# BarclayII/audiogan

Hardware: AMD Instinct MI355X
Metric: audio-samples/sec per G+D train step (8 kHz, 8192-sample clips) (higher is better)
Workload: dtype f32; 1 GPU; C2: full audiogan.py Conv1d/LSTM G + D, batch 64 per GPU, 8192-sample white-noise clips, frame_size 256 (T=32), canonical G+D step, adam, per-parameter clip d=1 g=0.1; global_batch=64, clip_len=8192, parallelism=dp1, launch=hipGraph replay (1 graph per step)

## Files before the change

audiogan_amd/csrc/conv_grad.hip:

```cpp
#include "common.h"

struct WgP {
  const float* sh;
  const float* lg;
  float* dw;
  int64_t sh_bs, sh_cs, lg_bs, lg_cs;
  int B, A, Lsh, C, Llg, K, s, p;
  int CK;
  int TC;
  int nchunk;
  int lgp;
  int maxch;
  int vec;
  float* part;
  int rb;
};

template <int TA, int TN, int WA, int WN>
__global__ __launch_bounds__(512) void conv_wgrad_kernel(const WgP p) {
  int bx = blockIdx.x, by = blockIdx.y, bz = blockIdx.z;
  const int gz_ = gridDim.z;
  {
    const int gx = gridDim.x, gy = gridDim.y, nwg = gx * gy * gz_;
    if (nwg >= 16) {
      const int lin = (bz * gy + by) * gx + bx;
      const int xi = lin & 7, q = nwg >> 3, r = nwg & 7;
      const int t = xi * q + (xi < r ? xi : r) + (lin >> 3);
      bx = t % gx; by = (t / gx) % gy; bz = t / (gx * gy);
    }
  }
  static_assert(WA * WN == 4, "4 compute waves");
  constexpr int AT = 32 * TA * WA, NT = 32 * TN * WN;
  constexpr int SP = AT + 1;
  extern __shared__ float smem[];
  const size_t bufsz = (size_t)p.TC * SP + (size_t)p.maxch * p.lgp;

  const int tid = threadIdx.x, lane = tid & 63, wid = tid >> 6;
  const int l31 = lane & 31, h = lane >> 5;
  const int cw = wid & 3;
  const int wa = cw / WN, wn = cw % WN;
  const int a0 = by * AT, ck0 = bx * NT;
  const int c_lo = ck0 / p.K;
  int c_hi = (ck0 + NT - 1) / p.K;
  if (c_hi >= p.C) c_hi = p.C - 1;
  const int nch = c_hi - c_lo + 1;
  const int span = p.s * (p.TC - 1) + p.K;
  const int total = p.B * p.nchunk;
  const int nmine = (total - bz + gz_ - 1) / gz_;

  auto stage = [&](int ch, int buf, int sw, int nsw) {
    float* shs = smem + buf * bufsz;
    float* lgs = shs + (size_t)p.TC * SP;
    const int b = ch / p.nchunk;
    const int t0 = (ch - b * p.nchunk) * p.TC;
    const float* sb = p.sh + (int64_t)b * p.sh_bs;
    const float* lb = p.lg + (int64_t)b * p.lg_bs;
    const int g0 = p.s * t0 - p.p;
    const int q4 = p.TC >> 2;
    const int stot = AT * q4, ltot = nch * span, step = nsw * 64;
    constexpr int US = 4, UL = 4;
    int se = sw * 64 + lane, le = se;
    while (se < stot || le < ltot) {
      f32x4 sv[US];
      float lv[UL];
#pragma unroll
      for (int u = 0; u < US; ++u) {
        const int e = se + u * step;
        sv[u] = f32x4{0.f, 0.f, 0.f, 0.f};
        if (e < stot) {
          const int r = e / q4, q = e - r * q4;
          const int a = a0 + r, tg = t0 + 4 * q;
          if (a < p.A) {
            const float* src = sb + (int64_t)a * p.sh_cs + tg;
            if (p.vec && tg + 3 < p.Lsh) {
              sv[u] = *reinterpret_cast<const f32x4*>(src);
            } else {
#pragma unroll
              for (int x = 0; x < 4; ++x)
                if (tg + x < p.Lsh) sv[u][x] = src[x];
            }
          }
        }
      }
#pragma unroll
      for (int u = 0; u < UL; ++u) {
        const int e = le + u * step;
        lv[u] = 0.f;
        if (e < ltot) {
          const int r = e / span, i = e - r * span;
          const int g = g0 + i;
          if (g >= 0 && g < p.Llg) lv[u] = lb[(int64_t)(c_lo + r) * p.lg_cs + g];
        }
      }
      if (p.rb) {
#pragma unroll
        for (int u = 0; u < US; ++u) sv[u] = ag_rbf4_if(sv[u], 1);
#pragma unroll
        for (int u = 0; u < UL; ++u) lv[u] = ag_rbf(lv[u]);
      }
#pragma unroll
      for (int u = 0; u < US; ++u) {
        const int e = se + u * step;
        if (e < stot) {
          const int r = e / q4, q = e - r * q4;
#pragma unroll
          for (int x = 0; x < 4; ++x) shs[(4 * q + x) * SP + r] = sv[u][x];
        }
      }
#pragma unroll
      for (int u = 0; u < UL; ++u) {
        const int e = le + u * step;
        if (e < ltot) {
          const int r = e / span, i = e - r * span;
          lgs[r * p.lgp + i] = lv[u];
        }
      }
      se += US * step;
      le += UL * step;
    }
  };

  if (nmine > 0) stage(bz, 0, wid, 8);
  __syncthreads();

  if (__builtin_amdgcn_readfirstlane(threadIdx.x) >= 256) {
    __builtin_amdgcn_s_setprio(2);
    constexpr int FS = 4, FL = 5;
    const int shift = (((-p.p) % 4) + 4) % 4;
    const int PR = (shift + span + 3) / 4;
    const int q4 = p.TC >> 2;
    const int stot = AT * q4, ltot4 = nch * PR;
    const bool fastp = p.vec && (p.Lsh % p.TC == 0) && ((p.s * p.TC) % 4 == 0) && (p.Llg % 4 == 0) && p.Llg >= 4 &&
                       (p.lg_cs % 4 == 0) && (p.lg_bs % 4 == 0) && (((uintptr_t)p.lg & 15) == 0) &&
                       stot <= FS * 256 && ltot4 <= FL * 256 && (int64_t)AT * p.sh_cs < (1 << 30) &&
                       (int64_t)p.maxch * p.lg_cs < (1 << 30);
    int ssrc[FS], sl[FS], lsrc[FL], li0[FL], lrow[FL];
    if (fastp) {
#pragma unroll
      for (int u = 0; u < FS; ++u) {
        const int e = cw * 64 + lane + u * 256;
        const int r = e / q4, q = e - r * q4;
        const bool ok = e < stot && a0 + r < p.A;
        ssrc[u] = ok ? (int)((a0 + r) * p.sh_cs) + 4 * q : 0;
        sl[u] = e < stot ? (4 * q) * SP + r : -1;
        if (e < stot && !ok) ssrc[u] = -1;
      }
#pragma unroll
      for (int u = 0; u < FL; ++u) {
        const int e = cw * 64 + lane + u * 256;
        const int r = e / PR, m = e - r * PR;
        const bool ok = e < ltot4;
        lsrc[u] = ok ? (int)((c_lo + r) * p.lg_cs) + 4 * m : 0;
        li0[u] = ok ? 4 * m - shift : -(1 << 20);
        lrow[u] = r * p.lgp;
      }
    }
    int ci = 0;
    if (fastp) {
      for (; ci < nmine; ++ci) {
        if (ci + 1 < nmine) {
          const int ch = bz + (ci + 1) * gz_;
          const int b = ch / p.nchunk;
          const int t0 = (ch - b * p.nchunk) * p.TC;
          const int g0 = p.s * t0 - p.p;
          float* shs = smem + ((ci + 1) & 1) * bufsz;
          float* lgs = shs + (size_t)p.TC * SP;
          const float* sbase = p.sh + (int64_t)b * p.sh_bs + t0;
          const float* lrow0 = p.lg + (int64_t)b * p.lg_bs;
          f32x4 sv[FS], lv[FL];
          bool lok[FL];
#pragma unroll
          for (int u = 0; u < FS; ++u) sv[u] = *reinterpret_cast<const f32x4*>(sbase + max(ssrc[u], 0));
#pragma unroll
          for (int u = 0; u < FL; ++u) {
            const int gp = g0 + li0[u];
            lok[u] = gp >= 0 && gp + 3 < p.Llg;
            lv[u] = *reinterpret_cast<const f32x4*>(lrow0 + (lok[u] ? lsrc[u] + (g0 - shift) : 0));
          }
          if (p.rb) {
#pragma unroll
            for (int u = 0; u < FS; ++u) sv[u] = ag_rbf4_if(sv[u], 1);
#pragma unroll
            for (int u = 0; u < FL; ++u) lv[u] = ag_rbf4_if(lv[u], 1);
          }
#pragma unroll
          for (int u = 0; u < FS; ++u)
            if (sl[u] >= 0) {
#pragma unroll
              for (int x = 0; x < 4; ++x) shs[sl[u] + x * SP] = ssrc[u] < 0 ? 0.f : sv[u][x];
            }
#pragma unroll
          for (int u = 0; u < FL; ++u)
#pragma unroll
            for (int x = 0; x < 4; ++x) {
              const int i = li0[u] + x;
              if (i >= 0 && i < span) lgs[lrow[u] + i] = lok[u] ? lv[u][x] : 0.f;
            }
        }
        __syncthreads();
      }
    }
    for (; ci < nmine; ++ci) {
      if (ci + 1 < nmine) stage(bz + (ci + 1) * gz_, (ci + 1) & 1, cw, 4);
      __syncthreads();
    }
    return;
  }

  int joff[TN];
  bool jok[TN];
#pragma unroll
  for (int j = 0; j < TN; ++j) {
    const int ck = ck0 + wn * 32 * TN + 32 * j + l31;
    jok[j] = ck < p.CK;
    const int c = jok[j] ? ck / p.K : c_lo;
    const int k = jok[j] ? ck - c * p.K : 0;
    joff[j] = (c - c_lo) * p.lgp + k + p.s * h;
  }
  f32x16 acc[TA][TN];
#pragma unroll
  for (int i = 0; i < TA; ++i)
#pragma unroll
    for (int j = 0; j < TN; ++j)
#pragma unroll
      for (int e = 0; e < 16; ++e) acc[i][j][e] = 0.f;

  for (int ci = 0; ci < nmine; ++ci) {
    const float* shs = smem + (ci & 1) * bufsz;
    const float* lgs = shs + (size_t)p.TC * SP;
    const float* arow = shs + h * SP + wa * 32 * TA + l31;
    for (int t = 0; t < p.TC; t += 2) {
      float av[TA], bv[TN];
#pragma unroll
      for (int i = 0; i < TA; ++i) av[i] = arow[t * SP + 32 * i];
#pragma unroll
      for (int j = 0; j < TN; ++j) {
        const float bval = lgs[joff[j] + p.s * t];
        bv[j] = jok[j] ? bval : 0.f;
      }
#pragma unroll
      for (int i = 0; i < TA; ++i)
#pragma unroll
        for (int j = 0; j < TN; ++j)
          acc[i][j] = __builtin_amdgcn_mfma_f32_32x32x2f32(av[i], bv[j], acc[i][j], 0, 0, 0);
    }
    __syncthreads();
  }

#pragma unroll
  for (int i = 0; i < TA; ++i)
#pragma unroll
    for (int e = 0; e < 16; ++e) {
      const int a = a0 + wa * 32 * TA + 32 * i + (e & 3) + 8 * (e >> 2) + 4 * h;
      if (a >= p.A) continue;
#pragma unroll
      for (int j = 0; j < TN; ++j) {
        const int ck = ck0 + wn * 32 * TN + 32 * j + l31;
        if (ck >= p.CK) continue;
        p.part[((int64_t)bz * p.A + a) * p.CK + ck] = acc[i][j][e];
      }
    }
}

typedef short wbf16x8 __attribute__((ext_vector_type(8)));
typedef unsigned wu32x4 __attribute__((ext_vector_type(4)));
typedef unsigned wu32x2 __attribute__((ext_vector_type(2)));
#define WB_FS 8
#define WB_FL 5

template <int TA, int TN, int WA, int WN>
__global__ __launch_bounds__(512) void conv_wgrad_bf16_kernel(const WgP p) {
  int bx = blockIdx.x, by = blockIdx.y, bz = blockIdx.z;
  const int gz_ = gridDim.z;
  {
    const int gx = gridDim.x, gy = gridDim.y, nwg = gx * gy * gz_;
    if (nwg >= 16) {
      const int lin = (bz * gy + by) * gx + bx;
      const int xi = lin & 7, q = nwg >> 3, r = nwg & 7;
      const int t = xi * q + (xi < r ? xi : r) + (lin >> 3);
      bx = t % gx; by = (t / gx) % gy; bz = t / (gx * gy);
    }
  }
  static_assert(WA * WN == 4, "4 compute waves");
  constexpr int AT = 32 * TA * WA, NT = 32 * TN * WN;
  extern __shared__ float smem[];
  char* lds = reinterpret_cast<char*>(smem);
  const int SPB = p.TC * 2 + 16;
  const int LGPB = p.lgp;
  const size_t bufb = ((size_t)AT * SPB + (size_t)p.maxch * LGPB + 15) & ~(size_t)15;

  const int tid = threadIdx.x, lane = tid & 63, wid = tid >> 6;
  const int l31 = lane & 31, h = lane >> 5;
  const int cw = wid & 3;
  const int wa = cw / WN, wn = cw % WN;
  const int a0 = by * AT, ck0 = bx * NT;
  const int c_lo = ck0 / p.K;
  int c_hi = (ck0 + NT - 1) / p.K;
  if (c_hi >= p.C) c_hi = p.C - 1;
  const int nch = c_hi - c_lo + 1;
  const int span = p.s * (p.TC - 1) + p.K;
  const int total = p.B * p.nchunk;
  const int nmine = (total - bz + gz_ - 1) / gz_;

  if (__builtin_amdgcn_readfirstlane(threadIdx.x) >= 256) {
    __builtin_amdgcn_s_setprio(2);
    const int sl_ = cw * 64 + lane;
    const int shift = (((-p.p) % 4) + 4) % 4;
    const int PR = (shift + span + 3) / 4;
    const int q4 = p.TC >> 2;
    const int stot = AT * q4, ltot4 = nch * PR;
    int ssrc[WB_FS], sdst[WB_FS], lsrc[WB_FL], li0[WB_FL], lrow[WB_FL];
#pragma unroll
    for (int u = 0; u < WB_FS; ++u) {
      const int e = sl_ + u * 256;
      const int r = e / q4, q = e - r * q4;
      const bool ok = e < stot && a0 + r < p.A;
      ssrc[u] = ok ? (int)((a0 + r) * p.sh_cs) + 4 * q : -1;
      sdst[u] = e < stot ? r * SPB + 8 * q : -1;
    }
#pragma unroll
    for (int u = 0; u < WB_FL; ++u) {
      const int e = sl_ + u * 256;
      const int r = e / PR, m = e - r * PR;
      const bool ok = e < ltot4;
      lsrc[u] = ok ? (int)((c_lo + r) * p.lg_cs) + 4 * m : 0;
      li0[u] = ok ? 4 * m - shift : -(1 << 20);
      lrow[u] = r * LGPB;
    }
    f32x4 sv[WB_FS], lv[WB_FL];
    bool lok[WB_FL];
    auto loadc = [&](int cix) __attribute__((always_inline)) {
      const int ch = bz + cix * gz_;
      const int b = ch / p.nchunk;
      const int t0 = (ch - b * p.nchunk) * p.TC;
      const int g0 = p.s * t0 - p.p;
      const float* sbase = p.sh + (int64_t)b * p.sh_bs + t0;
      const float* lrow0 = p.lg + (int64_t)b * p.lg_bs;
#pragma unroll
      for (int u = 0; u < WB_FS; ++u) sv[u] = *reinterpret_cast<const f32x4*>(sbase + max(ssrc[u], 0));
#pragma unroll
      for (int u = 0; u < WB_FL; ++u) {
        const int gp = g0 + li0[u];
        lok[u] = gp >= 0 && gp + 3 < p.Llg;
        lv[u] = *reinterpret_cast<const f32x4*>(lrow0 + (lok[u] ? lsrc[u] + (g0 - shift) : 0));
      }
    };
    auto writec = [&](int buf) __attribute__((always_inline)) {
      char* shs = lds + buf * bufb;
      char* lgs = shs + (size_t)AT * SPB;
#pragma unroll
      for (int u = 0; u < WB_FS; ++u)
        if (sdst[u] >= 0) {
          wu32x2 w = {ag_pack_bf16(sv[u][0], sv[u][1]), ag_pack_bf16(sv[u][2], sv[u][3])};
          if (ssrc[u] < 0) w = wu32x2{0u, 0u};
          *reinterpret_cast<wu32x2*>(shs + sdst[u]) = w;
        }
#pragma unroll
      for (int u = 0; u < WB_FL; ++u)
#pragma unroll
        for (int x = 0; x < 4; ++x) {
          const int i = li0[u] + x;
          if (i >= 0 && i < span)
            *reinterpret_cast<unsigned short*>(lgs + lrow[u] + 2 * i) = lok[u] ? (unsigned short)ag_pack_bf16(lv[u][x], lv[u][x]) : (unsigned short)0;
        }
    };
    if (nmine > 0) {
      loadc(0);
      writec(0);
    }
    __builtin_amdgcn_sched_barrier(0);
    if (nmine > 1) loadc(1);
    __syncthreads();
    for (int ci = 0; ci < nmine; ++ci) {
      if (ci + 1 < nmine) writec((ci + 1) & 1);
      __builtin_amdgcn_sched_barrier(0);
      if (ci + 2 < nmine) loadc(ci + 2);
      __syncthreads();
    }
    return;
  }

  int joff[TN];
  bool jok[TN];
#pragma unroll
  for (int j = 0; j < TN; ++j) {
    const int ck = ck0 + wn * 32 * TN + 32 * j + l31;
    jok[j] = ck < p.CK;
    const int c = jok[j] ? ck / p.K : c_lo;
    const int k = jok[j] ? ck - c * p.K : 0;
    joff[j] = (c - c_lo) * LGPB + 2 * (k + p.s * 8 * h);
  }
  f32x16 acc[TA][TN];
#pragma unroll
  for (int i = 0; i < TA; ++i)
#pragma unroll
    for (int j = 0; j < TN; ++j)
#pragma unroll
      for (int e = 0; e < 16; ++e) acc[i][j][e] = 0.f;
  __syncthreads();
  const int s2 = 2 * p.s;
  for (int ci = 0; ci < nmine; ++ci) {
    const char* shs = lds + (ci & 1) * bufb;
    const char* lgs = shs + (size_t)AT * SPB;
    const char* arow = shs + (size_t)(wa * 32 * TA + l31) * SPB + 16 * h;
    for (int tb = 0; tb < p.TC; tb += 16) {
      wbf16x8 av[TA], bv[TN];
#pragma unroll
      for (int i = 0; i < TA; ++i) av[i] = *reinterpret_cast<const wbf16x8*>(arow + (size_t)32 * i * SPB + 2 * tb);
#pragma unroll
      for (int j = 0; j < TN; ++j) {
        const char* bp = lgs + joff[j] + s2 * tb;
        wu32x4 w;
#pragma unroll
        for (int e = 0; e < 4; ++e) {
          const unsigned lo = *reinterpret_cast<const unsigned short*>(bp + s2 * (2 * e));
          const unsigned hi = *reinterpret_cast<const unsigned short*>(bp + s2 * (2 * e + 1));
          w[e] = jok[j] ? (lo | (hi << 16)) : 0u;
        }
        bv[j] = __builtin_bit_cast(wbf16x8, w);
      }
#pragma unroll
      for (int i = 0; i < TA; ++i)
#pragma unroll
        for (int j = 0; j < TN; ++j)
          acc[i][j] = __builtin_amdgcn_mfma_f32_32x32x16_bf16(av[i], bv[j], acc[i][j], 0, 0, 0);
    }
    __syncthreads();
  }

#pragma unroll
  for (int i = 0; i < TA; ++i)
#pragma unroll
    for (int e = 0; e < 16; ++e) {
      const int a = a0 + wa * 32 * TA + 32 * i + (e & 3) + 8 * (e >> 2) + 4 * h;
      if (a >= p.A) continue;
#pragma unroll
      for (int j = 0; j < TN; ++j) {
        const int ck = ck0 + wn * 32 * TN + 32 * j + l31;
        if (ck >= p.CK) continue;
        p.part[((int64_t)bz * p.A + a) * p.CK + ck] = acc[i][j][e];
      }
    }
}

static int wgrad_slices(int A, int CK, int AT, int NT, int total) {
  const int gx = ag_cdiv(CK, NT), gy = ag_cdiv(A, AT);
  int gz = ag_cdiv(512, gx * gy);
  if (gz > total) gz = total;
  if (gz < 1) gz = 1;
  return gz;
}

template <int TA, int TN, int WA, int WN>
static int launch_wgrad_bf16(WgP& p, hipStream_t st, AgWs ws) {
  constexpr int AT = 32 * TA * WA, NT = 32 * TN * WN;
  p.TC = 64;
  if (p.Lsh % p.TC != 0 || !p.vec || (p.s * p.TC) % 4 != 0 || p.Llg % 4 != 0 || p.Llg < 4 || p.lg_cs % 4 != 0 ||
      p.lg_bs % 4 != 0 || (((uintptr_t)p.lg) & 15) != 0)
    return -1;
  p.nchunk = p.Lsh / p.TC;
  const int span = p.s * (p.TC - 1) + p.K;
  p.lgp = ag_roundup(2 * span, 4) + 4;
  p.maxch = (NT - 1) / p.K + 2;
  if (p.maxch > p.C) p.maxch = p.C;
  const int shift = (((-p.p) % 4) + 4) % 4;
  const int PR = (shift + span + 3) / 4;
  if (AT * (p.TC / 4) > WB_FS * 256 || p.maxch * PR > WB_FL * 256) return -1;
  if ((int64_t)AT * p.sh_cs >= (1 << 30) || (int64_t)p.C * p.lg_cs >= (1 << 30)) return -1;
  const size_t lds = 2 * (((size_t)AT * (p.TC * 2 + 16) + (size_t)p.maxch * p.lgp + 15) & ~(size_t)15);
  if (lds > 160 * 1024) return -1;
  const int gx = ag_cdiv(p.CK, NT), gy = ag_cdiv(p.A, AT);
  const int total = p.B * p.nchunk;
  int gz = wgrad_slices(p.A, p.CK, AT, NT, total);
  const int64_t n_out = (int64_t)p.A * p.CK;
  AG_REQUIRE(ws.p && ws.numel >= n_out, "%s: this reduction spans several workgroups and needs a workspace of >= %lld floats bound with ag_bind_workspace (sums are two-stage, in a fixed order; there is no float-atomic accumulation)", "ag_conv1d_wgrad", (long long)n_out);
  if ((int64_t)gz * n_out > ws.numel) gz = (int)(ws.numel / n_out);
  p.part = ws.p;
  auto kern = conv_wgrad_bf16_kernel<TA, TN, WA, WN>;
  if (lds > 64 * 1024)
    (void)hipFuncSetAttribute((const void*)kern, hipFuncAttributeMaxDynamicSharedMemorySize, (int)lds);
  static const AgKernelName name("conv_wgrad_bf16_kernel", {TA, TN, WA, WN});
  ag_note_kernel(name.s);
  hipLaunchKernelGGL(kern, dim3(gx, gy, gz), dim3(512), lds, st, p);
  AG_CHECK_LAUNCH("ag_conv1d_wgrad(bf16)");
  return ag_slab_reduce(p.part, gz, n_out, p.dw, 1, st);
}

template <int TA, int TN, int WA, int WN>
static int launch_wgrad(WgP& p, hipStream_t st, AgWs ws) {
  constexpr int AT = 32 * TA * WA, NT = 32 * TN * WN;
  if (p.rb) {
    const int rc = launch_wgrad_bf16<TA, TN, WA, WN>(p, st, ws);
    if (rc != -1) return rc;
  }
  p.TC = AT >= 128 ? 32 : 64;
  if (p.Lsh < p.TC) p.TC = ag_roundup(p.Lsh, 4);
  p.nchunk = ag_cdiv(p.Lsh, p.TC);
  const int span = p.s * (p.TC - 1) + p.K;
  p.lgp = span | 1;
  p.maxch = (NT - 1) / p.K + 2;
  if (p.maxch > p.C) p.maxch = p.C;
  const size_t lds = 2 * ((size_t)p.TC * (AT + 1) + (size_t)p.maxch * p.lgp) * sizeof(float);
  if (lds > 160 * 1024) {
    ag_set_error("conv wgrad: tile needs %zu B of LDS", lds);
    return AG_ERR_UNSUPPORTED;
  }
  const int gx = ag_cdiv(p.CK, NT), gy = ag_cdiv(p.A, AT);
  const int total = p.B * p.nchunk;
  int gz = wgrad_slices(p.A, p.CK, AT, NT, total);
  const int64_t n_out = (int64_t)p.A * p.CK;
  AG_REQUIRE(ws.p && ws.numel >= n_out, "%s: this reduction spans several workgroups and needs a workspace of >= %lld floats bound with ag_bind_workspace (sums are two-stage, in a fixed order; there is no float-atomic accumulation)", "ag_conv1d_wgrad", (long long)n_out);
  if ((int64_t)gz * n_out > ws.numel) gz = (int)(ws.numel / n_out);
  p.part = ws.p;
  auto kern = conv_wgrad_kernel<TA, TN, WA, WN>;
  if (lds > 64 * 1024)
    (void)hipFuncSetAttribute((const void*)kern, hipFuncAttributeMaxDynamicSharedMemorySize,
                              (int)lds);
  static const AgKernelName name("conv_wgrad_kernel", {TA, TN, WA, WN});
  ag_note_kernel(name.s);
  hipLaunchKernelGGL(kern, dim3(gx, gy, gz), dim3(512), lds, st, p);
  AG_CHECK_LAUNCH("ag_conv1d_wgrad");
  return ag_slab_reduce(p.part, gz, n_out, p.dw, 1, st);
}

template <int KMAX, int AG>
__global__ __launch_bounds__(256) void conv_c1_wgrad_kernel(const float* __restrict__ sh, int64_t sh_bs, int64_t sh_cs,
                                                            const float* __restrict__ lg, int64_t lg_bs,
                                                            float* __restrict__ dw, int B, int A, int Lsh, int Llg,
                                                            int K, int s, int p, int bper, float* __restrict__ part,
                                                            int rb) {
  __shared__ float red[4][AG * KMAX];
  const int a0 = blockIdx.y * AG;
  const int t = blockIdx.x * 256 + threadIdx.x;
  const int b0 = blockIdx.z * bper, b1 = min(B, b0 + bper);
  float acc[AG][KMAX];
#pragma unroll
  for (int i = 0; i < AG; ++i)
#pragma unroll
    for (int k = 0; k < KMAX; ++k) acc[i][k] = 0.f;
  if (t < Lsh) {
    const int q0 = s * t - p;
    for (int b = b0; b < b1; ++b) {
      const float* xr = lg + (int64_t)b * lg_bs;
      float win[KMAX];
#pragma unroll
      for (int k = 0; k < KMAX; ++k) {
        const int q = q0 + k;
        const float xv = xr[min(max(q, 0), Llg - 1)];
        win[k] = (k < K && q >= 0 && q < Llg) ? ag_rbf_if(xv, rb) : 0.f;
      }
      const float* dyr = sh + (int64_t)b * sh_bs + t;
#pragma unroll
      for (int i = 0; i < AG; ++i) {
        const float g = ag_rbf_if(dyr[(int64_t)min(a0 + i, A - 1) * sh_cs], rb);
#pragma unroll
        for (int k = 0; k < KMAX; ++k) acc[i][k] += g * win[k];
      }
    }
  }
#pragma unroll
  for (int i = 0; i < AG; ++i)
#pragma unroll
    for (int k = 0; k < KMAX; ++k) {
      const float v = ag_wave_sum(acc[i][k]);
      if ((threadIdx.x & 63) == 0) red[threadIdx.x >> 6][i * KMAX + k] = v;
    }
  __syncthreads();
  if (threadIdx.x < AG * KMAX) {
    const int i = threadIdx.x / KMAX, k = threadIdx.x % KMAX;
    if (k < K && a0 + i < A) {
      const float v = red[0][threadIdx.x] + red[1][threadIdx.x] + red[2][threadIdx.x] + red[3][threadIdx.x];
      part[((int64_t)(blockIdx.z * gridDim.x + blockIdx.x) * A + a0 + i) * K + k] = v;
    }
  }
}

extern "C" int ag_conv1d_wgrad(const float* sh, int64_t sh_bs, int64_t sh_cs, const float* lg,
                               int64_t lg_bs, int64_t lg_cs, float* dw, int B, int A, int Lsh, int C,
                               int Llg, int K, int stride, int pad, void* stream) {
  const AgWs ws = ag_ws_take();
  AG_REQUIRE(sh && lg && dw, "ag_conv1d_wgrad: null tensor");
  AG_REQUIRE(B > 0 && A > 0 && Lsh > 0 && C > 0 && Llg > 0 && K > 0 && stride > 0 && pad >= 0,
             "ag_conv1d_wgrad: bad shape");
  WgP p;
  p.sh = sh; p.lg = lg; p.dw = dw;
  p.sh_bs = sh_bs; p.sh_cs = sh_cs; p.lg_bs = lg_bs; p.lg_cs = lg_cs;
  p.B = B; p.A = A; p.Lsh = Lsh; p.C = C; p.Llg = Llg; p.K = K; p.s = stride; p.p = pad;
  p.CK = C * K;
  p.rb = ag_precision() == AG_PREC_BF16;
  p.vec = (((uintptr_t)sh & 15) == 0) && (sh_bs % 4 == 0) && (sh_cs % 4 == 0);
  hipStream_t st = (hipStream_t)stream;
  if (C == 1 && ws.p && ag_conv_c1_wgrad_slabs(B, A, Lsh, stride, K, nullptr) > 0 &&
      (((uintptr_t)sh & 15) == 0) && sh_bs % 4 == 0 && sh_cs % 4 == 0 &&
      ws.numel >= (int64_t)ag_conv_c1_wgrad_slabs(B, A, Lsh, stride, K, nullptr) * A * K &&
      ag_conv_c1_enabled()) {
    const int slabs = ag_conv_c1_wgrad_slabs(B, A, Lsh, stride, K, nullptr);
    const int rc = ag_conv_c1_wgrad(sh, sh_bs, sh_cs, lg, lg_bs, ws.p, B, A, Lsh, Llg, stride, K, pad, p.rb, st);
    if (rc != AG_OK) return rc;
    return ag_slab_reduce(ws.p, slabs, (int64_t)A * K, dw, 1, st);
  }
  if (C == 1 && K <= 8) {
    const int ag = 8;
    const int gx = ag_cdiv(Lsh, 256), gy = ag_cdiv(A, ag);
    int gz = ag_cdiv(512, gx * gy);
    if (gz > B) gz = B;
    if (gz < 1) gz = 1;
    AG_REQUIRE(ws.p && ws.numel >= (int64_t)gx * A * K, "%s: this reduction spans several workgroups and needs a workspace of >= %lld floats bound with ag_bind_workspace (sums are two-stage, in a fixed order; there is no float-atomic accumulation)", "ag_conv1d_wgrad", (long long)gx * A * K);
    if ((int64_t)gz * gx * A * K > ws.numel) gz = (int)(ws.numel / ((int64_t)gx * A * K));
    float* part = ws.p;
    const int bper = ag_cdiv(B, gz);
    gz = ag_cdiv(B, bper);
    ag_note_kernel("conv_c1_wgrad_kernel<8,8>");
    hipLaunchKernelGGL((conv_c1_wgrad_kernel<8, 8>), dim3(gx, gy, gz), dim3(256), 0, st, sh, sh_bs, sh_cs, lg, lg_bs,
                       dw, B, A, Lsh, Llg, K, stride, pad, bper, part, p.rb);
    AG_CHECK_LAUNCH("ag_conv1d_wgrad");
    return ag_slab_reduce(part, gx * gz, (int64_t)A * K, dw, 1, st);
  }
  if (A <= 32) return launch_wgrad<1, 1, 1, 4>(p, st, ws);
  if (A <= 64 || p.CK <= 64) return launch_wgrad<1, 1, 2, 2>(p, st, ws);
  return launch_wgrad<2, 2, 2, 2>(p, st, ws);
}

extern "C" int64_t ag_conv1d_wgrad_ws_numel(int B, int A, int Lsh, int C, int K) {
  if (C == 1 && K == 7) {
    const int64_t need = (int64_t)ag_conv_c1_wgrad_slabs(B, A, Lsh, 2, K, nullptr) * A * K;
    const int gx = ag_cdiv(Lsh, 256), gy = ag_cdiv(A, 8);
    int gz = ag_cdiv(512, gx * gy);
    if (gz > B) gz = B;
    if (gz < 1) gz = 1;
    const int64_t n2 = (int64_t)gz * gx * A * K;
    return n2 > need ? n2 : need;
  }
  if (C == 1 && K <= 8) {
    const int gx = ag_cdiv(Lsh, 256), gy = ag_cdiv(A, 8);
    int gz = ag_cdiv(512, gx * gy);
    if (gz > B) gz = B;
    if (gz < 1) gz = 1;
    return (int64_t)gz * gx * A * K;
  }
  const int CK = C * K;
  int AT, NT;
  if (A <= 32) { AT = 32; NT = 128; }
  else if (A <= 64 || CK <= 64) { AT = 64; NT = 64; }
  else { AT = 128; NT = 128; }
  int TC = AT >= 128 ? 32 : 64;
  if (Lsh < TC) TC = ag_roundup(Lsh, 4);
  const int total = B * ag_cdiv(Lsh, TC);
  return (int64_t)wgrad_slices(A, CK, AT, NT, total) * A * CK;
}

__global__ __launch_bounds__(256) void channel_sum_kernel(const float* __restrict__ dy, int64_t bs,
                                                          int64_t cs, float* __restrict__ db, int B,
                                                          int C, int L, int nsplit, float* __restrict__ part, int accumulate) {
  __shared__ float red[17];
  const int c = blockIdx.x;
  const int64_t total = (int64_t)B * L;
  float s = 0.f;
  for (int64_t i = (int64_t)blockIdx.y * 256 + threadIdx.x; i < total; i += (int64_t)nsplit * 256) {
    const int b = (int)(i / L);
    const int t = (int)(i - (int64_t)b * L);
    s += dy[(int64_t)b * bs + (int64_t)c * cs + t];
  }
  s = ag_block_sum(s, red);
  if (threadIdx.x == 0) {
    if (part) part[(int64_t)blockIdx.y * C + c] = s;
    else db[c] = accumulate ? db[c] + s : s;
  }
}

extern "C" int ag_channel_sum(const float* dy, int64_t bs, int64_t cs, float* db, int B, int C, int L, int accumulate,
                              void* stream) {
  const AgWs ws = ag_ws_take();
  AG_REQUIRE(dy && db && B > 0 && C > 0 && L > 0, "ag_channel_sum: bad args");
  int nsplit = (int)ag_cdiv64((int64_t)B * L, 256 * 16);
  const int cap = ag_cdiv(2048, C);
  if (nsplit > cap) nsplit = cap;
  if (nsplit < 1) nsplit = 1;
  float* part = nullptr;
  if (nsplit > 1) {
    AG_REQUIRE(ws.p && ws.numel >= 2 * (int64_t)C, "%s: this reduction spans several workgroups and needs a workspace of >= %lld floats bound with ag_bind_workspace (sums are two-stage, in a fixed order; there is no float-atomic accumulation)", "ag_channel_sum", (long long)2 * C);
    if ((int64_t)nsplit * C > ws.numel) nsplit = (int)(ws.numel / C);
    part = ws.p;
  }
  hipLaunchKernelGGL(channel_sum_kernel, dim3(C, nsplit), dim3(256), 0, (hipStream_t)stream, dy, bs,
                     cs, db, B, C, L, nsplit, part, accumulate);
  AG_CHECK_LAUNCH("ag_channel_sum");
  if (part) return ag_slab_reduce(part, nsplit, C, db, accumulate ? 1 : 0, (hipStream_t)stream);
  return AG_OK;
}

__global__ __launch_bounds__(256) void leaky_bwd_kernel(const float* __restrict__ dy, int64_t dy_bs,
                                                        int64_t dy_cs, const float* __restrict__ y,
                                                        int64_t y_bs, int64_t y_cs,
                                                        float* __restrict__ dp, int64_t dp_bs,
                                                        int64_t dp_cs, float* __restrict__ ad,
                                                        int64_t ad_bs, int64_t ad_cs,
                                                        const int64_t* __restrict__ lens,
                                                        float* __restrict__ bias_grad, int B, int C,
                                                        int L, int bper, float slope, float* __restrict__ part) {
  const int c = blockIdx.y;
  float bsum = 0.f;
  for (int b = blockIdx.z * bper; b < min(B, (int)(blockIdx.z + 1) * bper); ++b) {
    const int64_t lenb = lens ? lens[b] : (int64_t)1 << 60;
    const float* dyr = dy + (int64_t)b * dy_bs + (int64_t)c * dy_cs;
    const float* yr = y + (int64_t)b * y_bs + (int64_t)c * y_cs;
    float* dpr = dp + (int64_t)b * dp_bs + (int64_t)c * dp_cs;
    float* adr = ad ? ad + (int64_t)b * ad_bs + (int64_t)c * ad_cs : nullptr;
    for (int t = blockIdx.x * 256 + threadIdx.x; t < L; t += gridDim.x * 256) {
      float g = dyr[t];
      g = (yr[t] > 0.f) ? g : g * slope;
      if (t >= lenb) g = 0.f;
      dpr[t] = g;
      if (adr) adr[t] += g;
      bsum += g;
    }
  }
  if (bias_grad) {
    __shared__ float red[4];
    bsum = ag_wave_sum(bsum);
    if ((threadIdx.x & 63) == 0) red[threadIdx.x >> 6] = bsum;
    __syncthreads();
    if (threadIdx.x == 0) {
      const float v = red[0] + red[1] + red[2] + red[3];
      part[(int64_t)(blockIdx.z * gridDim.x + blockIdx.x) * C + c] = v;
    }
  }
}

extern "C" int ag_leaky_bwd(const float* dy, int64_t dy_bs, int64_t dy_cs, const float* y,
                            int64_t y_bs, int64_t y_cs, float* dpre, int64_t dp_bs, int64_t dp_cs,
                            float* add_into, int64_t ad_bs, int64_t ad_cs, const int64_t* lens_i64,
                            float* bias_grad, int B, int C, int L, float slope, void* stream) {
  const AgWs ws = ag_ws_take();
  AG_REQUIRE(dy && y && dpre && B > 0 && C > 0 && L > 0, "ag_leaky_bwd: bad args");
  AG_REQUIRE(B <= 65535 && C <= 65535, "ag_leaky_bwd: B or C > 65535");
  int gx = ag_cdiv(L, 256 * 4);
  if (gx < 1) gx = 1;
  int bper = 1;
  float* part = nullptr;
  if (bias_grad) {
    bper = (int)(((int64_t)gx * C * B) / 2048);
    if (bper < 8) bper = 8;
    if (bper > B) bper = B;
    AG_REQUIRE(ws.p && ws.numel >= (int64_t)gx * C, "%s: this reduction spans several workgroups and needs a workspace of >= %lld floats bound with ag_bind_workspace (sums are two-stage, in a fixed order; there is no float-atomic accumulation)", "ag_leaky_bwd", (long long)gx * C);
    const int64_t zmax = ws.numel / ((int64_t)gx * C);
    if (ag_cdiv(B, bper) > zmax) bper = ag_cdiv(B, (int)zmax);
    part = ws.p;
  }
  const int gz = ag_cdiv(B, bper);
  hipLaunchKernelGGL(leaky_bwd_kernel, dim3(gx, C, gz), dim3(256), 0, (hipStream_t)stream, dy, dy_bs,
                     dy_cs, y, y_bs, y_cs, dpre, dp_bs, dp_cs, add_into, ad_bs, ad_cs, lens_i64, bias_grad, B, C, L,
                     bper, slope, part);
  AG_CHECK_LAUNCH("ag_leaky_bwd");
  if (part) return ag_slab_reduce(part, gx * gz, C, bias_grad, 1, (hipStream_t)stream);
  return AG_OK;
}

#define O1_MAXK 9

#define O1_UC 8

template <int K>
__global__ __launch_bounds__(256) void conv_o1_fwd_vec_kernel(const float* __restrict__ x, int64_t x_bs, int64_t x_cs,
                                                              const float* __restrict__ w,
                                                              const float* __restrict__ bias, float* __restrict__ y,
                                                              int64_t y_bs, int C, int L, int act, float slope, int rb) {
  constexpr int P = (K - 1) / 2;
  const int b = blockIdx.y, lane = threadIdx.x & 63;
  const int t0 = (blockIdx.x * 256 + threadIdx.x) * 4;
  const bool live = t0 < L;
  const float* xb = x + (int64_t)b * x_bs + (live ? t0 : 0);
  float acc[4] = {0.f, 0.f, 0.f, 0.f};
  for (int c0 = 0; c0 < C; c0 += O1_UC) {
    f32x4 v[O1_UC];
    float hl[O1_UC][P], hr[O1_UC][P];
#pragma unroll
    for (int u = 0; u < O1_UC; ++u) {
      const int c = min(c0 + u, C - 1);
      const float* xc = xb + (int64_t)c * x_cs;
      v[u] = *reinterpret_cast<const f32x4*>(xc);
#pragma unroll
      for (int i = 0; i < P; ++i) {
        hl[u][i] = (lane == 0 && live) ? xc[max(-(int)(i + 1), -t0)] : 0.f;
        hr[u][i] = (lane == 63 && live) ? xc[min(4 + i, L - 1 - t0)] : 0.f;
      }
    }
#pragma unroll
    for (int u = 0; u < O1_UC; ++u) {
      if (c0 + u >= C) break;
      float win[4 + 2 * P];
#pragma unroll
      for (int j = 0; j < 4; ++j) win[P + j] = ag_rbf_if(v[u][j], rb);
#pragma unroll
      for (int i = 0; i < P; ++i) {
        const float l_ = __shfl_up(v[u][3 - i], 1, 64), r_ = __shfl_down(v[u][i], 1, 64);
        const float lv = (lane == 0) ? hl[u][i] : l_, rv = (lane == 63) ? hr[u][i] : r_;
        win[P - 1 - i] = (t0 - 1 - i >= 0) ? ag_rbf_if(lv, rb) : 0.f;
        win[P + 4 + i] = (t0 + 4 + i < L) ? ag_rbf_if(rv, rb) : 0.f;
      }
      const float* wc = w + (c0 + u) * K;
#pragma unroll
      for (int k = 0; k < K; ++k) {
        const float wk = ag_rbf_if(wc[k], rb);
#pragma unroll
        for (int j = 0; j < 4; ++j) acc[j] += wk * win[j + k];
      }
    }
  }
  if (!live) return;
  const float bo = bias ? bias[0] : 0.f;
  f32x4 o = {ag_apply_act(acc[0] + bo, act, slope), ag_apply_act(acc[1] + bo, act, slope),
             ag_apply_act(acc[2] + bo, act, slope), ag_apply_act(acc[3] + bo, act, slope)};
  *reinterpret_cast<f32x4*>(y + (int64_t)b * y_bs + t0) = o;
}

__global__ __launch_bounds__(256) void conv_o1_fwd_kernel(const float* __restrict__ x, int64_t x_bs, int64_t x_cs,
                                                          const float* __restrict__ w, const float* __restrict__ bias,
                                                          float* __restrict__ y, int64_t y_bs, int C, int L, int K,
                                                          int p, int act, float slope, int rb) {
  const int b = blockIdx.y;
  const int t0 = (blockIdx.x * 256 + threadIdx.x) * 4;
  if (t0 >= L) return;
  const float* xb = x + (int64_t)b * x_bs;
  float acc[4] = {0.f, 0.f, 0.f, 0.f};
  for (int c = 0; c < C; ++c) {
    const float* xc = xb + (int64_t)c * x_cs;
    float win[4 + O1_MAXK - 1];
#pragma unroll
    for (int i = 0; i < 4 + O1_MAXK - 1; ++i) {
      const int g = t0 + i - p;
      const float v = (i < 4 + K - 1) ? xc[min(max(g, 0), L - 1)] : 0.f;
      win[i] = (g >= 0 && g < L) ? ag_rbf_if(v, rb) : 0.f;
    }
#pragma unroll
    for (int k = 0; k < O1_MAXK; ++k) {
      if (k >= K) break;
      const float wk = ag_rbf_if(w[c * K + k], rb);
#pragma unroll
      for (int j = 0; j < 4; ++j) acc[j] += wk * win[j + k];
    }
  }
  const float bo = bias ? bias[0] : 0.f;
#pragma unroll
  for (int j = 0; j < 4; ++j)
    if (t0 + j < L) y[(int64_t)b * y_bs + t0 + j] = ag_apply_act(acc[j] + bo, act, slope);
}

__global__ __launch_bounds__(256) void conv_o1_bwdx_kernel(const float* __restrict__ dy, int64_t dy_bs,
                                                           const float* __restrict__ w, float* __restrict__ dx,
                                                           int64_t dx_bs, int64_t dx_cs, int C, int L, int K, int p,
                                                           int accumulate, int rb) {
  const int b = blockIdx.z, c = blockIdx.y;
  const int t0 = (blockIdx.x * 256 + threadIdx.x) * 4;
  if (t0 >= L) return;
  const float* dyb = dy + (int64_t)b * dy_bs;
  float win[4 + O1_MAXK - 1];
#pragma unroll
  for (int i = 0; i < 4 + O1_MAXK - 1; ++i) {
    const int g = t0 + p - (K - 1) + i;
    const float v = (i < 4 + K - 1) ? dyb[min(max(g, 0), L - 1)] : 0.f;
    win[i] = (g >= 0 && g < L) ? ag_rbf_if(v, rb) : 0.f;
  }
  float acc[4] = {0.f, 0.f, 0.f, 0.f};
#pragma unroll
  for (int k = 0; k < O1_MAXK; ++k) {
    if (k >= K) break;
    const float wk = ag_rbf_if(w[c * K + k], rb);
#pragma unroll
    for (int j = 0; j < 4; ++j) acc[j] += wk * win[j + (K - 1) - k];
  }
  float* d = dx + (int64_t)b * dx_bs + (int64_t)c * dx_cs;
  if (t0 + 3 < L && (((uintptr_t)(d + t0)) & 15) == 0) {
    f32x4 o = {acc[0], acc[1], acc[2], acc[3]};
    if (accumulate) o += *reinterpret_cast<const f32x4*>(d + t0);
    *reinterpret_cast<f32x4*>(d + t0) = o;
    return;
  }
#pragma unroll
  for (int j = 0; j < 4; ++j)
    if (t0 + j < L) d[t0 + j] = accumulate ? d[t0 + j] + acc[j] : acc[j];
}

__global__ __launch_bounds__(256) void conv_o1_wgrad_kernel(const float* __restrict__ dy, int64_t dy_bs,
                                                            const float* __restrict__ x, int64_t x_bs, int64_t x_cs,
                                                            float* __restrict__ dw, int B, int C, int L, int K, int p,
                                                            int bper, float* __restrict__ part, int rb) {
  __shared__ float red[17];
  const int c = blockIdx.y;
  const int t0 = (blockIdx.x * 256 + threadIdx.x) * 4;
  const int b0 = blockIdx.z * bper;
  const int b1 = min(B, b0 + bper);
  float acc[O1_MAXK];
#pragma unroll
  for (int k = 0; k < O1_MAXK; ++k) acc[k] = 0.f;
  if (t0 < L) {
    for (int b = b0; b < b1; ++b) {
      const float* dyb = dy + (int64_t)b * dy_bs;
      const float* xc = x + (int64_t)b * x_bs + (int64_t)c * x_cs;
      float g[4], win[4 + O1_MAXK - 1];
#pragma unroll
      for (int j = 0; j < 4; ++j) {
        const float v = dyb[min(t0 + j, L - 1)];
        g[j] = (t0 + j < L) ? ag_rbf_if(v, rb) : 0.f;
      }
#pragma unroll
      for (int i = 0; i < 4 + O1_MAXK - 1; ++i) {
        const int q = t0 + i - p;
        const float v = (i < 4 + K - 1) ? xc[min(max(q, 0), L - 1)] : 0.f;
        win[i] = (q >= 0 && q < L) ? ag_rbf_if(v, rb) : 0.f;
      }
#pragma unroll
      for (int k = 0; k < O1_MAXK; ++k) {
        if (k < K) {
#pragma unroll
          for (int j = 0; j < 4; ++j) acc[k] += g[j] * win[j + k];
        }
      }
    }
  }
#pragma unroll
  for (int k = 0; k < O1_MAXK; ++k) {
    if (k < K) {
      const float s = ag_block_sum(acc[k], red);
      if (threadIdx.x == 0) {
        part[((int64_t)(blockIdx.z * gridDim.x + blockIdx.x) * C + c) * K + k] = s;
      }
    }
  }
}

extern "C" int ag_conv1d_o1_fwd(const float* x, int64_t x_bs, int64_t x_cs, const float* w, const float* bias,
                                float* y, int64_t y_bs, int B, int C, int L, int K, int pad, int act, float slope,
                                void* stream) {
  AG_REQUIRE(x && w && y && B > 0 && C > 0 && L > 0 && K > 0 && K <= O1_MAXK && pad >= 0 && B <= 65535,
             "ag_conv1d_o1_fwd: bad args (needs stride 1, K <= 9)");
  AG_REQUIRE(L + 2 * pad - K + 1 == L, "ag_conv1d_o1_fwd: needs a length-preserving ('same') conv");
  const int rb_ = (int)(ag_precision() == AG_PREC_BF16);
  if (K == 3 && L % 4 == 0 && L >= 4 && x_bs % 4 == 0 && x_cs % 4 == 0 && y_bs % 4 == 0 &&
      (((uintptr_t)x | (uintptr_t)y) & 15) == 0) {
    hipLaunchKernelGGL((conv_o1_fwd_vec_kernel<3>), dim3(ag_cdiv(L, 1024), B), dim3(256), 0, (hipStream_t)stream, x, x_bs,
                       x_cs, w, bias, y, y_bs, C, L, act, slope, rb_);
    AG_CHECK_LAUNCH("ag_conv1d_o1_fwd");
    return AG_OK;
  }
  hipLaunchKernelGGL(conv_o1_fwd_kernel, dim3(ag_cdiv(L, 1024), B), dim3(256), 0, (hipStream_t)stream, x, x_bs, x_cs,
                     w, bias, y, y_bs, C, L, K, pad, act, slope, (int)(ag_precision() == AG_PREC_BF16));
  AG_CHECK_LAUNCH("ag_conv1d_o1_fwd");
  return AG_OK;
}

#define O1_CPB 16
// ... 128 lines not shown
```

Measured before the change: 30.88 million audio-samples/sec.

## Pipeline wgrad producer loads two chunks ahead and size split-K grid by occupancy

After: 31.19 million audio-samples/sec (median of 6 runs). No clear change (+1.0%).

```diff
diff --git a/audiogan_amd/csrc/conv_grad.hip b/audiogan_amd/csrc/conv_grad.hip
--- a/audiogan_amd/csrc/conv_grad.hip
+++ b/audiogan_amd/csrc/conv_grad.hip
@@ -1,4 +1,7 @@
 #include "common.h"
+
+#include <mutex>
+#include <vector>
 
 struct WgP {
   const float* sh;
@@ -121,7 +124,6 @@
   };
 
   if (nmine > 0) stage(bz, 0, wid, 8);
-  __syncthreads();
 
   if (__builtin_amdgcn_readfirstlane(threadIdx.x) >= 256) {
     __builtin_amdgcn_s_setprio(2);
@@ -134,74 +136,80 @@
                        (p.lg_cs % 4 == 0) && (p.lg_bs % 4 == 0) && (((uintptr_t)p.lg & 15) == 0) &&
                        stot <= FS * 256 && ltot4 <= FL * 256 && (int64_t)AT * p.sh_cs < (1 << 30) &&
                        (int64_t)p.maxch * p.lg_cs < (1 << 30);
+    if (!fastp) {
+      __syncthreads();
+      for (int ci = 0; ci < nmine; ++ci) {
+        if (ci + 1 < nmine) stage(bz + (ci + 1) * gz_, (ci + 1) & 1, cw, 4);
+        __syncthreads();
+      }
+      return;
+    }
     int ssrc[FS], sl[FS], lsrc[FL], li0[FL], lrow[FL];
-    if (fastp) {
-#pragma unroll
-      for (int u = 0; u < FS; ++u) {
-        const int e = cw * 64 + lane + u * 256;
-        const int r = e / q4, q = e - r * q4;
-        const bool ok = e < stot && a0 + r < p.A;
-        ssrc[u] = ok ? (int)((a0 + r) * p.sh_cs) + 4 * q : 0;
-        sl[u] = e < stot ? (4 * q) * SP + r : -1;
-        if (e < stot && !ok) ssrc[u] = -1;
-      }
+#pragma unroll
+    for (int u = 0; u < FS; ++u) {
+      const int e = cw * 64 + lane + u * 256;
+      const int r = e / q4, q = e - r * q4;
+      const bool ok = e < stot && a0 + r < p.A;
+      ssrc[u] = ok ? (int)((a0 + r) * p.sh_cs) + 4 * q : 0;
+      sl[u] = e < stot ? (4 * q) * SP + r : -1;
+      if (e < stot && !ok) ssrc[u] = -1;
+    }
+#pragma unroll
+    for (int u = 0; u < FL; ++u) {
+      const int e = cw * 64 + lane + u * 256;
+      const int r = e / PR, m = e - r * PR;
+      const bool ok = e < ltot4;
+      lsrc[u] = ok ? (int)((c_lo + r) * p.lg_cs) + 4 * m : 0;
+      li0[u] = ok ? 4 * m - shift : -(1 << 20);
+      lrow[u] = r * p.lgp;
+    }
+    f32x4 sv[FS], lv[FL];
+    bool lok[FL];
+    auto loadc = [&](int cix) __attribute__((always_inline)) {
+      const int ch = bz + cix * gz_;
+      const int b = ch / p.nchunk;
+      const int t0 = (ch - b * p.nchunk) * p.TC;
+      const int g0 = p.s * t0 - p.p;
+      const float* sbase = p.sh + (int64_t)b * p.sh_bs + t0;
+      const float* lrow0 = p.lg + (int64_t)b * p.lg_bs;
+#pragma unroll
+      for (int u = 0; u < FS; ++u) sv[u] = *reinterpret_cast<const f32x4*>(sbase + max(ssrc[u], 0));
 #pragma unroll
       for (int u = 0; u < FL; ++u) {
-        const int e = cw * 64 + lane + u * 256;
-        const int r = e / PR, m = e - r * PR;
-        const bool ok = e < ltot4;
-        lsrc[u] = ok ? (int)((c_lo + r) * p.lg_cs) + 4 * m : 0;
-        li0[u] = ok ? 4 * m - shift : -(1 << 20);
-        lrow[u] = r * p.lgp;
-      }
-    }
-    int ci = 0;
-    if (fastp) {
-      for (; ci < nmine; ++ci) {
-        if (ci + 1 < nmine) {
-          const int ch = bz + (ci + 1) * gz_;
-          const int b = ch / p.nchunk;
-          const int t0 = (ch - b * p.nchunk) * p.TC;
-          const int g0 = p.s * t0 - p.p;
-          float* shs = smem + ((ci + 1) & 1) * bufsz;
-          float* lgs = shs + (size_t)p.TC * SP;
-          const float* sbase = p.sh + (int64_t)b * p.sh_bs + t0;
-          const float* lrow0 = p.lg + (int64_t)b * p.lg_bs;
-          f32x4 sv[FS], lv[FL];
-          bool lok[FL];
-#pragma unroll
-          for (int u = 0; u < FS; ++u) sv[u] = *reinterpret_cast<const f32x4*>(sbase + max(ssrc[u], 0));
-#pragma unroll
-          for (int u = 0; u < FL; ++u) {
-            const int gp = g0 + li0[u];
-            lok[u] = gp >= 0 && gp + 3 < p.Llg;
-            lv[u] = *reinterpret_cast<const f32x4*>(lrow0 + (lok[u] ? lsrc[u] + (g0 - shift) : 0));
-          }
-          if (p.rb) {
-#pragma unroll
-            for (int u = 0; u < FS; ++u) sv[u] = ag_rbf4_if(sv[u], 1);
-#pragma unroll
-            for (int u = 0; u < FL; ++u) lv[u] = ag_rbf4_if(lv[u], 1);
-          }
-#pragma unroll
-          for (int u = 0; u < FS; ++u)
-            if (sl[u] >= 0) {
-#pragma unroll
-              for (int x = 0; x < 4; ++x) shs[sl[u] + x * SP] = ssrc[u] < 0 ? 0.f : sv[u][x];
-            }
-#pragma unroll
-          for (int u = 0; u < FL; ++u)
-#pragma unroll
-            for (int x = 0; x < 4; ++x) {
-              const int i = li0[u] + x;
-              if (i >= 0 && i < span) lgs[lrow[u] + i] = lok[u] ? lv[u][x] : 0.f;
-            }
+        const int gp = g0 + li0[u];
+        lok[u] = gp >= 0 && gp + 3 < p.Llg;
+        lv[u] = *reinterpret_cast<const f32x4*>(lrow0 + (lok[u] ? lsrc[u] + (g0 - shift) : 0));
+      }
+    };
+    auto writec = [&](int buf) __attribute__((always_inline)) {
+      float* shs = smem + buf * bufsz;
+      float* lgs = shs + (size_t)p.TC * SP;
+      if (p.rb) {
+#pragma unroll
+        for (int u = 0; u < FS; ++u) sv[u] = ag_rbf4_if(sv[u], 1);
+#pragma unroll
+        for (int u = 0; u < FL; ++u) lv[u] = ag_rbf4_if(lv[u], 1);
+      }
+#pragma unroll
+      for (int u = 0; u < FS; ++u)
+        if (sl[u] >= 0) {
+#pragma unroll
+          for (int x = 0; x < 4; ++x) shs[sl[u] + x * SP] = ssrc[u] < 0 ? 0.f : sv[u][x];
         }
-        __syncthreads();
-      }
-    }
-    for (; ci < nmine; ++ci) {
-      if (ci + 1 < nmine) stage(bz + (ci + 1) * gz_, (ci + 1) & 1, cw, 4);
+#pragma unroll
+      for (int u = 0; u < FL; ++u)
+#pragma unroll
+        for (int x = 0; x < 4; ++x) {
+          const int i = li0[u] + x;
+          if (i >= 0 && i < span) lgs[lrow[u] + i] = lok[u] ? lv[u][x] : 0.f;
+        }
+    };
+    if (nmine > 1) loadc(1);
+    __syncthreads();
+    for (int ci = 0; ci < nmine; ++ci) {
+      if (ci + 1 < nmine) writec((ci + 1) & 1);
+      __builtin_amdgcn_sched_barrier(0);
+      if (ci + 2 < nmine) loadc(ci + 2);
       __syncthreads();
     }
     return;
@@ -224,6 +232,7 @@
     for (int j = 0; j < TN; ++j)
 #pragma unroll
       for (int e = 0; e < 16; ++e) acc[i][j][e] = 0.f;
+  __syncthreads();
 
   for (int ci = 0; ci < nmine; ++ci) {
     const float* shs = smem + (ci & 1) * bufsz;
@@ -443,7 +452,7 @@
     }
 }
 
-static int wgrad_slices(int A, int CK, int AT, int NT, int total) {
+static int wgrad_slices_bf16(int A, int CK, int AT, int NT, int total) {
   const int gx = ag_cdiv(CK, NT), gy = ag_cdiv(A, AT);
   int gz = ag_cdiv(512, gx * gy);
   if (gz > total) gz = total;
@@ -471,7 +480,7 @@
   if (lds > 160 * 1024) return -1;
   const int gx = ag_cdiv(p.CK, NT), gy = ag_cdiv(p.A, AT);
   const int total = p.B * p.nchunk;
-  int gz = wgrad_slices(p.A, p.CK, AT, NT, total);
+  int gz = wgrad_slices_bf16(p.A, p.CK, AT, NT, total);
   const int64_t n_out = (int64_t)p.A * p.CK;
   AG_REQUIRE(ws.p && ws.numel >= n_out, "%s: this reduction spans several workgroups and needs a workspace of >= %lld floats bound with ag_bind_workspace (sums are two-stage, in a fixed order; there is no float-atomic accumulation)", "ag_conv1d_wgrad", (long long)n_out);
   if ((int64_t)gz * n_out > ws.numel) gz = (int)(ws.numel / n_out);
@@ -486,16 +495,76 @@
   return ag_slab_reduce(p.part, gz, n_out, p.dw, 1, st);
 }
 
-template <int TA, int TN, int WA, int WN>
+template <int TA_, int TN_, int WA_, int WN_>
+struct WgForm {
+  static constexpr int TA = TA_, TN = TN_, WA = WA_, WN = WN_;
+  static constexpr int AT = 32 * TA * WA, NT = 32 * TN * WN;
+};
+
+template <class F>
+static auto wgrad_with_form(int A, int CK, F&& f) {
+  if (A <= 32) return f(WgForm<1, 1, 1, 4>{});
+  if (A <= 64 || CK <= 64) return f(WgForm<1, 1, 2, 2>{});
+  return f(WgForm<2, 2, 2, 2>{});
+}
+
+struct WgOcc { int dev; const void* kern; size_t lds; int per_cu, n_cu; };
+static int wgrad_occupancy(const void* kern, size_t lds, int* n_cu) {
+  static std::mutex mu;
+  static std::vector<WgOcc> cache;
+  int dev = 0;
+  if (hipGetDevice(&dev) != hipSuccess) return 0;
+  std::lock_guard<std::mutex> lock(mu);
+  for (const WgOcc& o : cache)
+    if (o.dev == dev && o.kern == kern && o.lds == lds) {
+      *n_cu = o.n_cu;
+      return o.per_cu;
+    }
+  WgOcc o{dev, kern, lds, 0, 0};
+  if (lds > 64 * 1024) (void)hipFuncSetAttribute(kern, hipFuncAttributeMaxDynamicSharedMemorySize, (int)lds);
+  if (hipDeviceGetAttribute(&o.n_cu, hipDeviceAttributeMultiprocessorCount, dev) != hipSuccess || o.n_cu < 1 ||
+      hipOccupancyMaxActiveBlocksPerMultiprocessor(&o.per_cu, kern, 512, lds) != hipSuccess || o.per_cu < 1) {
+    (void)hipGetLastError();
+    return 0;
+  }
+  cache.push_back(o);
+  *n_cu = o.n_cu;
+  return o.per_cu;
+}
+
+struct WgPlan {
+  int TC, nchunk, gx, gy, gz;
+};
+
+template <class Form>
+static WgPlan wgrad_plan(int B, int A, int Lsh, int C, int K) {
+  constexpr int AT = Form::AT, NT = Form::NT;
+  WgPlan pl;
+  pl.TC = AT >= 128 ? 32 : 64;
+  if (Lsh < pl.TC) pl.TC = ag_roundup(Lsh, 4);
+  pl.nchunk = ag_cdiv(Lsh, pl.TC);
+  pl.gx = ag_cdiv(C * K, NT);
+  pl.gy = ag_cdiv(A, AT);
+  int maxch = (NT - 1) / K + 2;
+  if (maxch > C) maxch = C;
+  const size_t lds = 2 * ((size_t)pl.TC * (AT + 1) + (size_t)maxch * ((pl.TC - 1 + K) | 1)) * sizeof(float);
+  int n_cu = 0;
+  int per_cu = wgrad_occupancy((const void*)conv_wgrad_kernel<Form::TA, Form::TN, Form::WA, Form::WN>, lds, &n_cu);
+  if (per_cu > 2) per_cu = 2;
+  const int total = B * pl.nchunk;
+  pl.gz = per_cu > 0 ? (per_cu * n_cu) / (pl.gx * pl.gy) : 0;
+  if (pl.gz > total) pl.gz = total;
+  if (pl.gz < 1 && per_cu > 0) pl.gz = 1;
+  return pl;
+}
+
+template <class Form>
 static int launch_wgrad(WgP& p, hipStream_t st, AgWs ws) {
-  constexpr int AT = 32 * TA * WA, NT = 32 * TN * WN;
-  if (p.rb) {
-    const int rc = launch_wgrad_bf16<TA, TN, WA, WN>(p, st, ws);
-    if (rc != -1) return rc;
-  }
-  p.TC = AT >= 128 ? 32 : 64;
-  if (p.Lsh < p.TC) p.TC = ag_roundup(p.Lsh, 4);
-  p.nchunk = ag_cdiv(p.Lsh, p.TC);
+  constexpr int TA = Form::TA, TN = Form::TN, WA = Form::WA, WN = Form::WN;
+  constexpr int AT = Form::AT, NT = Form::NT;
+  const WgPlan pl = wgrad_plan<Form>(p.B, p.A, p.Lsh, p.C, p.K);
+  p.TC = pl.TC;
+  p.nchunk = pl.nchunk;
   const int span = p.s * (p.TC - 1) + p.K;
   p.lgp = span | 1;
   p.maxch = (NT - 1) / p.K + 2;
@@ -505,9 +574,11 @@
     ag_set_error("conv wgrad: tile needs %zu B of LDS", lds);
     return AG_ERR_UNSUPPORTED;
   }
-  const int gx = ag_cdiv(p.CK, NT), gy = ag_cdiv(p.A, AT);
-  const int total = p.B * p.nchunk;
-  int gz = wgrad_slices(p.A, p.CK, AT, NT, total);
+  if (pl.gz < 1) {
+    ag_set_error("conv wgrad: the device's CU count / the kernel's occupancy could not be queried");
+    return AG_ERR_LAUNCH;
+  }
+  int gz = pl.gz;
   const int64_t n_out = (int64_t)p.A * p.CK;
   AG_REQUIRE(ws.p && ws.numel >= n_out, "%s: this reduction spans several workgroups and needs a workspace of >= %lld floats bound with ag_bind_workspace (sums are two-stage, in a fixed order; there is no float-atomic accumulation)", "ag_conv1d_wgrad", (long long)n_out);
   if ((int64_t)gz * n_out > ws.numel) gz = (int)(ws.numel / n_out);
@@ -518,9 +589,22 @@
                               (int)lds);
   static const AgKernelName name("conv_wgrad_kernel", {TA, TN, WA, WN});
   ag_note_kernel(name.s);
-  hipLaunchKernelGGL(kern, dim3(gx, gy, gz), dim3(512), lds, st, p);
+  hipLaunchKernelGGL(kern, dim3(pl.gx, pl.gy, gz), dim3(512), lds, st, p);
   AG_CHECK_LAUNCH("ag_conv1d_wgrad");
   return ag_slab_reduce(p.part, gz, n_out, p.dw, 1, st);
+}
+
+static int launch_wgrad_bf16_any(WgP& p, hipStream_t st, AgWs ws) {
+  if (p.A <= 32) return launch_wgrad_bf16<1, 1, 1, 4>(p, st, ws);
+  if (p.A <= 64 || p.CK <= 64) return launch_wgrad_bf16<1, 1, 2, 2>(p, st, ws);
+  return launch_wgrad_bf16<2, 2, 2, 2>(p, st, ws);
+}
+static int wgrad_bf16_slabs(int B, int A, int Lsh, int CK) {
+  int AT, NT;
+  if (A <= 32) { AT = 32; NT = 128; }
+  else if (A <= 64 || CK <= 64) { AT = 64; NT = 64; }
+  else { AT = 128; NT = 128; }
+  return Lsh % 64 == 0 ? wgrad_slices_bf16(A, CK, AT, NT, B * (Lsh / 64)) : 0;
 }
 
 template <int KMAX, int AG>
@@ -616,9 +700,11 @@
     AG_CHECK_LAUNCH("ag_conv1d_wgrad");
     return ag_slab_reduce(part, gx * gz, (int64_t)A * K, dw, 1, st);
   }
-  if (A <= 32) return launch_wgrad<1, 1, 1, 4>(p, st, ws);
-  if (A <= 64 || p.CK <= 64) return launch_wgrad<1, 1, 2, 2>(p, st, ws);
-  return launch_wgrad<2, 2, 2, 2>(p, st, ws);
+  if (p.rb) {
+    const int rc = launch_wgrad_bf16_any(p, st, ws);
+    if (rc != -1) return rc;
+  }
+  return wgrad_with_form(A, p.CK, [&](auto form) { return launch_wgrad<decltype(form)>(p, st, ws); });
 }
 
 extern "C" int64_t ag_conv1d_wgrad_ws_numel(int B, int A, int Lsh, int C, int K) {
@@ -639,14 +725,12 @@
     return (int64_t)gz * gx * A * K;
   }
   const int CK = C * K;
-  int AT, NT;
-  if (A <= 32) { AT = 32; NT = 128; }
-  else if (A <= 64 || CK <= 64) { AT = 64; NT = 64; }
-  else { AT = 128; NT = 128; }
-  int TC = AT >= 128 ? 32 : 64;
-  if (Lsh < TC) TC = ag_roundup(Lsh, 4);
-  const int total = B * ag_cdiv(Lsh, TC);
-  return (int64_t)wgrad_slices(A, CK, AT, NT, total) * A * CK;
+  int64_t gz = wgrad_with_form(A, CK, [&](auto form) { return wgrad_plan<decltype(form)>(B, A, Lsh, C, K).gz; });
+  if (ag_precision() == AG_PREC_BF16) {
+    const int gb = wgrad_bf16_slabs(B, A, Lsh, CK);
+    if (gb > gz) gz = gb;
+  }
+  return gz * A * CK;
 }
 
 __global__ __launch_bounds__(256) void channel_sum_kernel(const float* __restrict__ dy, int64_t bs,
```
